# izhengfan/se2lam

Hardware: AMD Instinct MI355X
Metric: BA GN-iters/s (200 KF, 20k pts) (higher is better)
Workload: dtype f64; 1 GPU; globalBA-window 200 KF / 20000 landmarks / 119817 EdgeSE2XYZ + 199 PreEdgeSE2, LM optimize(10) (config 4 formulation, SURVEY D3); parallelism=single GPU

## Files before the change

### include/se2gpu.h

```cpp
#ifndef SE2GPU_H
#define SE2GPU_H

#include <stddef.h>
#include <stdint.h>

#ifdef __cplusplus
extern "C" {
#endif

#define SE2GPU_OK 0
#define SE2GPU_ERR_INVALID (-1)
#define SE2GPU_ERR_NO_DEVICE (-2)
#define SE2GPU_ERR_HIP (-3)
#define SE2GPU_ERR_CAPACITY (-4)
#define SE2GPU_ERR_STATE (-5)

const char* se2gpu_last_error(void);
int se2gpu_device_count(void);
const char* se2gpu_version(void);

typedef struct se2gpu_orb se2gpu_orb;

typedef struct se2gpu_orb_params {
    int32_t nfeatures;
// ... 247 lines not shown
                                  int* n_local, int32_t* ref_kfs, int* n_ref, int32_t* local_mps, int* n_mps);

int se2gpu_ba_initialize(se2gpu_ba* h);
int se2gpu_ba_set_edge_level(se2gpu_ba* h, int edge, int level);
int se2gpu_ba_reset_estimates(se2gpu_ba* h);
int se2gpu_ba_reset_estimates_batch(se2gpu_ba** handles, int count);

#define SE2GPU_BA_LM 0
#define SE2GPU_BA_GN 1
int se2gpu_ba_optimize(se2gpu_ba* h, int iters, int mode, const volatile uint8_t* stop_flag, int verbose,
                       se2gpu_ba_stats* stats);
int se2gpu_ba_optimize_batch(se2gpu_ba** handles, int count, int iters, int mode, const volatile uint8_t* stop_flag,
                             se2gpu_ba_stats* stats);
int se2gpu_ba_last_batch_path(void);
int se2gpu_ba_get_se2(se2gpu_ba* h, int id, double xyt[3]);
int se2gpu_ba_get_xyz(se2gpu_ba* h, int id, double xyz[3]);
int se2gpu_ba_get_all(se2gpu_ba* h, double* poses , double* lms );
double se2gpu_ba_chi2(se2gpu_ba* h);

int se2gpu_ba_debug_reduced_system(se2gpu_ba* h, double lambda, double* S, double* bs);
int se2gpu_ba_debug_solve(se2gpu_ba* h, double lambda, double* x, int* factor_ok);
int se2gpu_ba_debug_solver_path(const se2gpu_ba* h);
int se2gpu_ba_debug_linearize_counts(const se2gpu_ba* h, int* runs, int* skips, long long* twin_bytes);
int se2gpu_ba_debug_pool_sizes(int out2[2]);
int se2gpu_ba_debug_chol_verify(se2gpu_ba* h, unsigned long long* counts2, unsigned long long* records, int cap);
int se2gpu_ba_debug_solve_plan(int P, int D, const uint8_t* pattern, int allow_nd, int* nsys, int* nbc, int* depth, int* ntask,
                               int* ndep, int32_t* pose_off, int32_t* tasks4, int task_cap, int32_t* deps, int dep_cap);
int se2gpu_ba_debug_solve_plan_tile(int P, int D, const uint8_t* pattern, int allow_nd, int tile, int* nsys, int* nbc, int* depth, int* ntask,
                                    int* ndep, int32_t* pose_off, int32_t* tasks4, int task_cap, int32_t* deps, int dep_cap);
int se2gpu_ba_debug_solve_plan_neager(int P, int D, const uint8_t* pattern, int allow_nd, int tile, int32_t* neager, int cap);
int se2gpu_ba_debug_plan_neager(se2gpu_ba* h, int* nsys, int* permuted, int* ntask, int32_t* neager, int cap);

int se2gpu_triangulate(int n, const se2gpu_keypoint* kps_ref, const se2gpu_keypoint* kps_cur, int n_cur,
                       int32_t* match_idx, const uint8_t* has_observation, const float* P_ref, const float* P_cur,
                       const float* Ocam, float lower_depth, float upper_depth, int min_degree, float* pos_out,
                       uint8_t* good_parallax, int* n_good, int* n_tracked_old);

typedef struct se2gpu_track se2gpu_track;
int se2gpu_track_create(se2gpu_track** out);
void se2gpu_track_destroy(se2gpu_track* h);
int se2gpu_track_fundamental_mask(se2gpu_track* h, const float* pt1, const float* pt2, int n, uint8_t* mask,
                                  int* n_inliers);
int se2gpu_track_remove_outliers(se2gpu_track* h, const se2gpu_keypoint* kps1, int n1, const se2gpu_keypoint* kps2,
                                 int n2, int32_t* matches, int* n_inliers);
int se2gpu_track_last_ransac(const se2gpu_track* h, int info[4]);
int se2gpu_track_set_stream(se2gpu_track* h, void* hip_stream);
// ... 131 lines not shown
```

### se2lam_amd/capi.py

```python
from __future__ import annotations

import ctypes as C
import os

import numpy as np

HERE = os.path.dirname(os.path.abspath(__file__))
LIB_PATH = os.path.join(HERE, "lib", "libse2gpu.so")

OK = 0
ERR_INVALID, ERR_NO_DEVICE, ERR_HIP, ERR_CAPACITY, ERR_STATE = -1, -2, -3, -4, -5


class Se2GpuError(RuntimeError):
    def __init__(self, code, msg):
        super().__init__(f"se2gpu error {code}: {msg}")
        self.code = code


class Keypoint(C.Structure):
    _fields_ = [("x", C.c_float), ("y", C.c_float), ("size", C.c_float), ("angle", C.c_float),
                ("response", C.c_float), ("octave", C.c_int32), ("class_id", C.c_int32)]


# ... 145 lines not shown
    "se2gpu_ba_add_edge_se3": (_I, [_VP, _I, _I, _PD, _PD]),
    "se2gpu_ba_add_edge_xyz2uv": (_I, [_VP, _I, _I, _PD, _D, _D]),
    "se2gpu_ba_get_se3": (_I, [_VP, _I, _PD]),
    "se2gpu_ba_edge_chi2": (_I, [_VP, _PD, _I]),
    "se2gpu_map_update_local_graph": (_I, [C.POINTER(MapView), _I, _I, _VP, C.POINTER(_I), _VP, C.POINTER(_I), _VP, C.POINTER(_I)]),
    "se2gpu_sparsify_se3xyz": (_I, [_I, _VP, _VP, _VP, _VP, _VP, _VP, _VP, _VP, _VP]),
    "se2gpu_feat_edge_batch": (_I, [_I, _I, _I, _I, _VP, _VP, _D, _D, _D, _VP, _VP, _VP, _VP, _D, _D, _VP, _VP, _VP, _VP, _VP,
                                    _VP, _VP, _VP]),
    "se2gpu_ba_initialize": (_I, [_VP]),
    "se2gpu_ba_set_edge_level": (_I, [_VP, _I, _I]),
    "se2gpu_ba_reset_estimates": (_I, [_VP]),
    "se2gpu_ba_reset_estimates_batch": (_I, [_VP, _I]),
    "se2gpu_ba_optimize": (_I, [_VP, _I, _I, _PU8, _I, C.POINTER(BaStats)]),
    "se2gpu_ba_optimize_batch": (_I, [C.POINTER(_VP), _I, _I, _I, _PU8, C.POINTER(BaStats)]),
    "se2gpu_ba_last_batch_path": (_I, []),
    "se2gpu_ba_get_se2": (_I, [_VP, _I, _PD]),
    "se2gpu_ba_get_xyz": (_I, [_VP, _I, _PD]),
    "se2gpu_ba_get_all": (_I, [_VP, _PD, _PD]),
    "se2gpu_ba_chi2": (_D, [_VP]),
    "se2gpu_ba_debug_reduced_system": (_I, [_VP, _D, _PD, _PD]),
    "se2gpu_ba_debug_solve": (_I, [_VP, _D, _PD, C.POINTER(C.c_int)]),
    "se2gpu_ba_debug_solver_path": (_I, [_VP]),
    "se2gpu_ba_debug_linearize_counts": (_I, [_VP, C.POINTER(C.c_int), C.POINTER(C.c_int), C.POINTER(C.c_longlong)]),
    "se2gpu_ba_debug_chol_verify": (_I, [_VP, _VP, _VP, _I]),
    "se2gpu_ba_debug_pool_sizes": (_I, [_VP]),
    "se2gpu_ba_debug_solve_plan": (_I, [_I, _I, _VP, _I, _VP, _VP, _VP, _VP, _VP, _VP, _VP, _I, _VP, _I]),
    "se2gpu_ba_debug_solve_plan_tile": (_I, [_I, _I, _VP, _I, _I, _VP, _VP, _VP, _VP, _VP, _VP, _VP, _I, _VP, _I]),
    "se2gpu_ba_debug_solve_plan_neager": (_I, [_I, _I, _VP, _I, _I, _VP, _I]),
    "se2gpu_ba_debug_plan_neager": (_I, [_VP, C.POINTER(C.c_int), C.POINTER(C.c_int), C.POINTER(C.c_int), _VP, _I]),
    "se2gpu_triangulate": (_I, [_I, _VP, _VP, _I, _VP, _VP, _VP, _VP, _VP, C.c_float, C.c_float, _I, _VP, _VP,
                           C.POINTER(C.c_int), C.POINTER(C.c_int)]),
    "se2gpu_track_create": (_I, [C.POINTER(_VP)]),
    "se2gpu_track_destroy": (None, [_VP]),
    "se2gpu_track_fundamental_mask": (_I, [_VP, _VP, _VP, _I, _VP, C.POINTER(C.c_int)]),
    "se2gpu_track_remove_outliers": (_I, [_VP, _VP, _I, _VP, _I, _VP, C.POINTER(C.c_int)]),
    "se2gpu_track_last_ransac": (_I, [_VP, _VP]),
    "se2gpu_track_set_stream": (_I, [_VP, _VP]),
    "se2gpu_track_stream": (_VP, [_VP]),
    "se2gpu_track_sync": (_I, [_VP]),
    "se2gpu_track_loop_verify_batch_device": (_I, [_VP, _VP, _VP, _I, _I, _VP, _VP, _VP, _VP, _I, _VP, _VP, _VP, _VP]),
    "se2gpu_plane_motion_prior": (_I, [_VP, _VP, _D, _D, _D, _VP, _VP]),
    "se2gpu_track_pose_ba": (_I, [_VP, _VP, _VP, _VP, _I, _VP, _VP, _VP, _D, _D, _D, _D, _I, _VP, C.POINTER(BaStats)]),
    "se2gpu_track_triangulate": (_I, [_VP, _I, _VP, _VP, _I, _VP, _VP, _VP, _VP, _VP, C.c_float, C.c_float, _I, _VP, _VP,
                                 C.POINTER(C.c_int), C.POINTER(C.c_int)]),
    "se2gpu_ba_reduce_buffer_doubles": (_SZ, [_VP, _I]),
    "se2gpu_ba_exchange_doubles": (_SZ, [_I]),
# ... 214 lines not shown
```

### se2lam_amd/csrc/ba.hip

```cpp
#include <algorithm>
#include <atomic>
#include <chrono>
#include <cmath>
#include <cstdlib>
#include <functional>
#include <limits>
#include <mutex>
#include <thread>
#include <memory>
#include <unordered_map>

#include "common.h"
#include "se3_math.h"
#include "ba_device.h"
#include "ba3_device.h"
#include "ba_window.h"

using namespace se2gpu;
using namespace se2gpu::badev;

namespace {



// ... 1395 lines not shown
                                                     const int* __restrict__ col_src) {
    if (ctl && ctl->done) return;
    const int r = blockIdx.x * 4 + threadIdx.x / 64;
    const int lane = threadIdx.x & 63;
    if (r >= n) return;
    const double* y = A + (size_t)n * ld;
    double acc = 0.0;
    for (int c = r + lane; c < n; c += 64) acc += R[(size_t)r * ld + c] * y[c];
    acc = wave_sum(acc);
    const int dst = col_src ? col_src[r] : r;
    if (lane == 0 && dst >= 0) x[dst] = acc;
}

struct TrialEnd {
    double* out;
    volatile double* mail;
    double seq;
    BaCtl* ctl;
    const volatile int* stop;
    int step;
    int decide;
    int notify;
    int spec;
};

struct FinArgs {
    int enabled, nblk, P, O, root;
    const uint8_t* fixed;
    const double* xp;
    const double* bp;
    const double* poses;
    double* poses_trial;
    const int* o_i;
    const int* o_j;
    const double* o_meas;
    const double* o_info;
    unsigned* counter;
    TrialEnd te;
};
__device__ void finish_trial(const FinArgs& fin, const double* part, double lambda, double* fsp);

struct SpecArgs {
    RecSet set[2];
    double *Hpp_e, *bp_e;
};

// ... 169 lines not shown
        for (int i = 0; i < kBlock / 64; ++i) { c += sm[0][i]; s += sm[1][i]; }
        if (a.fin.enabled) {
            store_agent(a.part + 2 * bx, d2_t{c, s});
            asm volatile("s_waitcnt vmcnt(0)" ::: "memory");
            __hip_atomic_fetch_add(a.fin.counter, 1u, __ATOMIC_RELAXED, __HIP_MEMORY_SCOPE_AGENT);
        } else {
            a.part[2 * bx] = c;
            a.part[2 * bx + 1] = s;
        }
    }
    if (LIN && spec)
        lin_landmark<true>(l, sub, beg, end, a.L, hll, bsum, lambda_spec, keep, wr.W, a.sp.Hpp_e, a.sp.bp_e, wr.Hll, wr.bl, wr.Ainv,
                           wr.zeta, wr.Dg);
}
template <bool LIN>
__global__ __launch_bounds__(kBlock) void k_update(UpdArgs a) {
    d_update<LIN>(blockIdx.x, a);
}

__global__ void k_ctl_clear_error(BaCtl* __restrict__ ctl) {
    ctl->error = 0;
    ctl->done = 0;
}

__device__ inline void post_ctl(const BaCtl* c, volatile double* mail, double seq, int tid, int nthr) {
    constexpr int kWords = (int)(sizeof(BaCtl) / 8);
    const double* src = reinterpret_cast<const double*>(c);
    for (int i = tid; i < kWords; i += nthr) mail[8 + i] = src[i];
}

__device__ inline void end_slot(BaCtl* ctl, volatile double* mail, bool post, int tid, int nthr, bool step) {
    if (!step) return;
    if (tid == 0) ctl->seq += 1.0;
    __syncthreads();
    if (post && mail) {
        __threadfence();
        post_ctl(ctl, mail, 0.0, tid, nthr);
        __threadfence_system();
        __syncthreads();
        if (tid == 0) mail[kMailSeq] = ctl->seq;
    }
}


struct TrialState { bool live, est_b; double lambda; };
__device__ __forceinline__ TrialState trial_open(const TrialEnd& t, double lambda) {
// ... 24 lines not shown
    __syncthreads();
    if (threadIdx.x == 0)
        for (int w = 1; w < nw; ++w) {
            chi += sm[w];
            scale += sm[nw + w];
        }
}

__device__ __forceinline__ bool trial_decide(const TrialEnd& t, double chi, double scale, double fail, bool stopped, bool records) {
    BaCtl* ctl = t.ctl;
    volatile double* mail = t.mail;
    t.out[0] = chi; t.out[1] = scale; t.out[3] = 0;
    if (!t.step) t.out[2] = 0;
    if (ctl && t.decide) {
        if (!t.step) {
            lm_begin(ctl, chi, stopped);
        } else {
            const double sc[3] = {chi, scale, fail};
            const int sel0 = ctl->sel;
            const bool speculated = t.spec && ctl->it + 1 < ctl->iters;
            const double lambda_spec = lm_lambda_spec(ctl->lambda, ctl->mode);
            lm_advance(ctl, sc, stopped);
            if (records && !ctl->error) lm_records_advance(ctl, speculated, sel0, lambda_spec);
        }
        return (ctl->done || t.notify) && mail;
    }
    if (mail && !ctl) {
        mail[0] = chi;
        mail[1] = scale;
        mail[2] = fail;
        __threadfence_system();
        mail[3] = t.seq;
    }
    return false;
}

__device__ __forceinline__ void trial_close(const TrialEnd& t, const int* post) {
    if (!(t.ctl && t.decide)) return;
    __syncthreads();
    end_slot(t.ctl, t.mail, *post != 0, threadIdx.x, blockDim.x, t.step != 0);
}

__device__ __forceinline__ void se2_pose_stage(const FinArgs& fin, const double* poses, double* poses_trial, double lambda,
                                               bool step, double* sp, double& scale) {
    for (int p = threadIdx.x; p < fin.P; p += blockDim.x) {
        double x = poses[3 * p], y = poses[3 * p + 1], th = poses[3 * p + 2];
// ... 966 lines not shown
    hipEvent_t join_event = nullptr;
    hipStream_t join_stream = nullptr;
    bool own_pending = false;
    int P = 0, L = 0, E = 0, O = 0, nblk = 0, nparts = 0;
    int ld = 0;
    bool host_solve = false;
    DevBuf<double> poses0, lms0, poses_a, poses_b, lms_a, lms_b;
    double *poses = nullptr, *poses_t = nullptr, *lms = nullptr, *lms_t = nullptr;
    DevBuf<uint8_t> fixed;
    DevBuf<int> lm_ptr, e_kf, e_lm, pose_ptr, pose_edges, podo_ptr, podo_item, o_i, o_j;
    DevBuf<int> blk_a, blk_b, blk_ptr, pair_i, pair_j, blk_odo;
    DevBuf<int4> grp;
    int nwg_off = 0, grp_cap_wg = 0;
    DevBuf<uint8_t> garena;
    DevBuf<int> plan_np, plan_base, plan_key0, plan_key1, plan_idx, plan_hist, plan_offs, plan_out, plan_tsum, plan_toff;
    DevBuf<int2> plan_st0, plan_st1;
    bool odo_fallback = false;
    bool odo_self_loop = false;
    DevBuf<double> e_uv, e_info, o_meas, o_info;
    DevBuf<double> Hpl, Hpp_e, bp_e, Hll, bl, Dinv, z, Y, Dg, Hpp, bp, Oii, Ojj, Oij, obi, obj;
    DevBuf<double> red_own, xp, part, scal, diag3, Rinv;
    DevBuf<double> rec_twin;
    bool run_spec = false;
    DevBuf<double> red_packed;
    DevBuf<int4> chol_tasks;
    DevBuf<int> chol_deps;
    DevBuf<int> chol_neager;
    DevBuf<int> pose_off;
    DevBuf<int> col_src;
    std::vector<int> h_pose_off;
    DevBuf<uint8_t> plan_nz;
    DevBuf<double> plan_nzd;
    PinBuf<uint8_t> h_plan_nz;
    DevBuf<uint8_t> solver_arena;
    int nsys = 0;
    int solve_depth = 0;
    DevBuf<unsigned> chol_flags;
    DevBuf<unsigned long long> chol_head;
    DevBuf<unsigned long long> chol_vfy;
    DevBuf<int> plan_place;
    DevBuf<unsigned> fin_counter;
    DevBuf<unsigned long long> l0_acc;
    int chol_ntask = 0;
    struct GraphSlot { int iters = -1, mode = -1; hipGraphExec_t exec = nullptr; unsigned long stamp = 0; };
    static constexpr int kGraphSlots = 3;
    GraphSlot graphs[kGraphSlots];
    unsigned long graph_clock = 0;
    void drop_graphs() {
        for (auto& g : graphs) {
            if (g.exec) (void)hipGraphExecDestroy(g.exec);
            g = GraphSlot{};
        }
    }
    double dev_seq = 0;
    DevBuf<long long> chol_trace;
    bool chol_steps = false;
    bool chol_faulted = false;
    bool chol_fallback = false;
    double* red = nullptr;
    PinBuf<double> h_red, h_x, h_scal;
    double* h_mail = nullptr;
    double* d_mail = nullptr;
    volatile int* h_stop = nullptr;
    int* d_stop = nullptr;
    uint64_t mail_seq = 0;
    DevBuf<BaCtl> ctl;
    int run_mode = SE2GPU_BA_LM, run_iters = 0, run_enqueued = 0;
// ... 1132 lines not shown
            hipLaunchKernelGGL(k_plan_place, dim3(kPackRuns), dim3(128), 0, st, nblk, h->blk_a.p, h->blk_b.p, h->blk_ptr.p, start,
                               h->grp.p, cap_wg, gpw);
        } else {
            hipLaunchKernelGGL(k_plan_pack, dim3(1), dim3(256), 0, st, nblk, h->blk_a.p, h->blk_b.p, h->blk_ptr.p, h->grp.p,
                               cap_wg, h->plan_out.p, gpw);
        }
        SE2_HIP(hipGetLastError());
        SE2_CHECK(h->h_scal.reserve(8 + (size_t)h->world));
        SE2_HIP(hipMemcpyAsync(h->h_scal.p, h->plan_out.p, sizeof(int), hipMemcpyDeviceToHost, st));
        lap("plan kernels enqueued");
    }
    sent = big_off;
    SE2_CHECK(stage_range(big_off, big_end, copy_stream));
    SE2_HIP(hipEventRecord(h->ev_copy1, copy_stream));
    lap("measurements staged");
    SE2_HIP(hipStreamWaitEvent(st, h->ev_copy1, 0));
    SE2_CHECK(h->fin_counter.reserve(1));
    SE2_HIP(hipMemsetAsync(h->fin_counter.p, 0, sizeof(unsigned), st));
    SE2_CHECK(h->l0_acc.reserve(2));
    SE2_HIP(hipMemsetAsync(h->l0_acc.p, 0, 2 * sizeof(unsigned long long), st));
    SE2_HIP(hipMemsetAsync(h->ctl.p, 0, sizeof(BaCtl), st));
    h->dev_seq = 0;
    h->drop_graphs();
    SE2_CHECK(h->h_x.reserve(n));
    SE2_CHECK(h->h_scal.reserve(8 + (size_t)h->world));
    if (!h->h_mail) {
        SE2_HIP(hipHostMalloc((void**)&h->h_mail, kMailDoubles * sizeof(double), hipHostMallocMapped | hipHostMallocCoherent));
        std::memset(h->h_mail, 0, kMailDoubles * sizeof(double));
        SE2_HIP(hipHostGetDevicePointer((void**)&h->d_mail, h->h_mail, 0));
        h->h_stop = reinterpret_cast<volatile int*>(h->h_mail + kMailStop);
        h->d_stop = reinterpret_cast<int*>(h->d_mail + kMailStop);
    }
    ((volatile double*)h->h_mail)[kMailSeq] = 0.0;
    h->poses = h->poses_a.p; h->poses_t = h->poses_b.p;
    h->lms = h->lms_a.p; h->lms_t = h->lms_b.p;
    SE2_HIP(hipMemcpyAsync(h->poses, h->poses0.p, (size_t)ps * P * 8, hipMemcpyDeviceToDevice, st));
    if (L) SE2_HIP(hipMemcpyAsync(h->lms, h->lms0.p, 3 * (size_t)L * 8, hipMemcpyDeviceToDevice, st));
    if (pattern_early) SE2_HIP(hipEventSynchronize(h->ev_pat));
    else SE2_HIP(hipStreamSynchronize(st));
    lap(pattern_early ? "pattern" : "synchronise");
    {
        std::vector<uint8_t> pat;
        if (nd_possible) {
            const uint8_t* nz = device_plan ? h->h_plan_nz.p : pl.blk_nz.data();
            pat.assign((size_t)P * P, 0);
            for (int a = 0; a < P; ++a) {
// ... 112 lines not shown
    if (i < np) poses[i] = poses0[i];
    if (i < nl) lms[i] = lms0[i];
}
__global__ __launch_bounds__(256) void k_reset_batch(const ResetItem* __restrict__ items) {
    const ResetItem it = items[blockIdx.y];
    const unsigned stride = gridDim.x * 256, t0 = blockIdx.x * 256 + threadIdx.x;
    for (unsigned i = t0; i < it.np; i += stride) it.dst_p[i] = it.src_p[i];
    for (unsigned i = t0; i < it.nl; i += stride) it.dst_l[i] = it.src_l[i];
}

struct Bufs {
    const BaCtl* c;
    double *pa, *pb, *la, *lb;
};
inline Bufs bufs(se2gpu_ba* h, bool ctl) {
    if (ctl) return Bufs{h->ctl.p, h->poses_a.p, h->poses_b.p, h->lms_a.p, h->lms_b.p};
    return Bufs{nullptr, h->poses, h->poses_t, h->lms, h->lms_t};
}

bool ba_env_speculate() {
    static const bool on = env_flag("SE2GPU_BA_SPECULATE", true);
    return on;
}
bool ba_env_open() {
    static const bool on = env_flag("SE2GPU_BA_OPEN", true);
    return on;
}
bool ba_opens_fused(const se2gpu_ba* h) {
    return ba_env_open() && h->model == 0 && !h->allreduce && !h->comm && h->L > 0 && !h->odo_fallback;
}
RecSet rec_own(const se2gpu_ba* h) { return RecSet{h->Hpl.p, h->Dg.p, h->Hll.p, h->bl.p, h->Dinv.p, h->z.p}; }
RecSet rec_twin(const se2gpu_ba* h) {
    if (!h->rec_twin.p || h->model) return RecSet{};
    const size_t E = (size_t)h->E, L = (size_t)h->L;
    double* p = h->rec_twin.p;
    RecSet r;
    r.W = p; p += 9 * E + 1;
    r.Dg = p; p += 12 * E + 1;
    r.Hll = p; p += 6 * L + 1;
    r.bl = p; p += 3 * L + 1;
    r.Ainv = p; p += 6 * L + 1;
    r.zeta = p;
    return r;
}
int ba_reserve_twin(se2gpu_ba* h) { return h->rec_twin.reserve(21 * (size_t)h->E + 18 * (size_t)h->L + 6); }

// ... 13 lines not shown
    return PoseReduceArgs{h->P, h->pose_ptr.p, h->pose_edges.p, h->Hpp_e.p, h->bp_e.p, h->podo_ptr.p, h->podo_item.p, h->Oii.p,
                          h->Ojj.p, h->obi.p, h->obj.p, h->Hpp.p, h->bp.p};
}
MaxdiagArgs maxdiag_args(se2gpu_ba* h, int dpp, int stride9, BaCtl* ctl) {
    return MaxdiagArgs{h->L, h->Hll.p, h->P, stride9 ? h->Hpp.p : h->diag3.p, h->fixed.p, h->scal.p, dpp, stride9, ctl};
}
Reduce2Args reduce2_args(se2gpu_ba* h, const Bufs& B, double lambda, const RecSet& alt) {
    return Reduce2Args{h->P, h->ld, h->nwg_off, lambda, h->root, h->grp.p, h->blk_a.p, h->blk_b.p, h->pair_i.p, h->pair_j.p,
                       h->blk_odo.p, h->Hpl.p, h->Dg.p, h->fixed.p, h->pose_ptr.p, h->pose_edges.p, h->podo_ptr.p, h->podo_item.p,
                       h->o_i.p, h->o_j.p, h->o_meas.p, h->o_info.p, B.pa, h->red, h->bp.p, B.c, B.pb, &h->ctl.p->epoch,
                       h->pose_off.p, h->nsys, alt.W, alt.Dg};
}
CholArgs chol_args(se2gpu_ba* h, const BaCtl* ctl, int skip, unsigned long long* head, bool verify) {
    const int n = h->nsys, ld = h->ld;
    const int nt = ld / kNB, nbc = (n + kNB - 1) / kNB;
    double* YU = h->Rinv.p + 2 * (size_t)nt * nbc * kSlabs * kSlabDoubles;
    unsigned* flagA = h->chol_flags.p;
    return CholArgs{h->red, h->Rinv.p, YU, ld, n, nbc, h->chol_tasks.p + skip, h->chol_deps.p, h->chol_neager.p + skip, h->col_src.p,
                    flagA, flagA + kSlabs * (size_t)nt * nbc, &h->ctl.p->epoch, ba_scal(h) + 2, h->chol_trace.p, ctl, h->xp.p,
                    verify ? h->chol_vfy.p : nullptr, head, h->chol_ntask - skip};
}
TrialEnd trial_end(se2gpu_ba* h, const Bufs& B, int step, int decide, int notify, double seq, bool lin = false, bool post = true) {
    return TrialEnd{ba_scal(h), post ? h->d_mail : nullptr, seq, B.c ? h->ctl.p : nullptr,
                    B.c ? (const volatile int*)h->d_stop : nullptr, step, decide, notify, lin ? 1 : 0};
}
FinArgs fin_args(se2gpu_ba* h, const Bufs& B, const double* xp, const TrialEnd& te) {
    return FinArgs{1, (int)upd_grid(h).x, h->P, h->O, h->root, h->fixed.p, xp, h->bp.p, B.pa, B.pb,
                   h->o_i.p, h->o_j.p, h->o_meas.p, h->o_info.p, h->fin_counter.p, te};
}
UpdArgs upd_args(se2gpu_ba* h, const Bufs& B, double lambda, const double* xp, const FinArgs& fin, bool lin = false) {
    return UpdArgs{h->cam, h->L, lambda, h->lm_ptr.p, h->e_kf.p, h->e_uv.p, h->e_info.p, B.pa, h->fixed.p, B.la, xp, h->z.p, h->Hpl.p,
                   h->bl.p, B.lb, h->part.p, B.c, B.pb, fin, h->Dinv.p,
                   lin ? SpecArgs{{rec_own(h), rec_twin(h)}, h->Hpp_e.p, h->bp_e.p} : SpecArgs{}};
}

inline const double* prior_hess(const se2gpu_ba* h) { return h->model == 2 ? h->ph.p : h->prior_info.p; }
inline Edges6 edges6(const se2gpu_ba* h) {
    if (h->model == 2) return Edges6{h->pg_edges, h->pe_i.p, h->pe_j.p, h->pe_meas.p, h->pe_info.p};
    return Edges6{h->O, h->o_i.p, h->o_j.p, h->o_meas.p, h->o_info.p};
}
inline dim3 terms6_grid(const se2gpu_ba* h) { return grid1((size_t)h->P + h->O, 64); }
Lin3Args lin3_args(se2gpu_ba* h, const Bufs& B, double lambda) {
    return Lin3Args{h->cam3, h->L, h->lm_ptr.p, h->e_kf.p, h->e_uv.p, h->e_info.p, B.pa, h->fixed.p, B.la, h->Hpl.p, h->Hpp_e.p,
                    h->bp_e.p, h->Hll.p, h->bl.p, lambda, h->Dinv.p, h->z.p, h->Y.p, h->Dg.p, B.c, B.pb, B.lb};
}
Terms6Args terms6_args(se2gpu_ba* h, const Bufs& B) {
    return Terms6Args{h->P, h->O, B.pa, h->fixed.p, h->prior_has.p, h->prior_meas.p, h->prior_info.p, h->ph.p, h->pb.p, h->slot_a.p,
// ... 323 lines not shown
    };
    if (first && ba_opens_fused(h)) {
        const OpenArgs oa = open_args(h, B, lm, seq);
        if (lm) {
            SE2_LAUNCH(h->prof, st, "k_open", k_open<false>, open_grid(h, oa, true), dim3(kBlock), 0, oa);
            SE2_CHECK(ba_lambda_init(h, &oa.fin));
            SE2_CHECK(ba_reduce(h, 0.0, 3, true));
        } else {
            SE2_LAUNCH(h->prof, st, "k_open", k_open<true>, open_grid(h, oa, false), dim3(kBlock), 0, oa);
            SE2_CHECK(ba_reduce(h, 0.0, 0, true));
        }
        SE2_HIP(hipGetLastError());
    } else if (first) {
        SE2_CHECK(evaluate(false, false));
        if (lm) {
            SE2_CHECK(ba_linearize(h, -1.0, true));
            SE2_CHECK(ba_lambda_init(h));
            SE2_CHECK(ba_reduce(h, 0.0, 3, true));
        } else {
            SE2_CHECK(ba_linearize(h, 0.0, true));
            SE2_CHECK(ba_reduce(h, 0.0, 0, true));
        }
    } else {
        if (know_retry != 1) SE2_CHECK(ba_linearize(h, 0.0, true));
        SE2_CHECK(ba_reduce(h, 0.0, !lm ? 0 : know_retry == 0 ? 0 : know_retry == 1 ? 3 : (h->model ? 2 : 0), true));
    }
    SE2_CHECK(ba_allreduce_system(h));
    SE2_CHECK(ba_solve(h, true));
    SE2_CHECK(evaluate(true, notify));
    return SE2GPU_OK;
}


template <typename Args>
struct Packed {
    int nblk;
    Args args;
};
template <typename Args, void (*Body)(unsigned, const Args&), int BS>
__global__ __launch_bounds__(BS) void k_batched(const Packed<Args>* __restrict__ p) {
    if ((int)blockIdx.x >= p[blockIdx.y].nblk) return;
    const Args a = p[blockIdx.y].args;
    Body(blockIdx.x, a);
}
template <typename Args, void (*Body)(unsigned, const Args&), int BS>
__global__ __launch_bounds__(BS) void k_batched_xcd(const Packed<Args>* __restrict__ p) {
    const unsigned nb = gridDim.x, nw8 = gridDim.y & ~7u;
// ... 892 lines not shown
    return SE2GPU_OK;
}

int se2gpu_ba_debug_pool_sizes(int out2[2]) {
    SE2_REQUIRE(out2, SE2GPU_ERR_INVALID, "debug_pool_sizes: NULL argument");
    { LeasePool<PlanSet>& p = LeasePool<PlanSet>::get(); std::lock_guard<std::mutex> g(p.mu); out2[0] = (int)p.idle.size(); }
    { LeasePool<ResetScratch>& p = LeasePool<ResetScratch>::get(); std::lock_guard<std::mutex> g(p.mu); out2[1] = (int)p.idle.size(); }
    return SE2GPU_OK;
}

int se2gpu_ba_debug_solver_path(const se2gpu_ba* h) {
    if (!h || !h->initialized) return -1;
    return h->host_solve ? 3 : h->chol_fallback ? 2 : h->chol_steps ? 1 : 0;
}

int se2gpu_ba_debug_linearize_counts(const se2gpu_ba* h, int* runs, int* skips, long long* twin_bytes) {
    SE2_REQUIRE(h && h->initialized, SE2GPU_ERR_STATE, "debug_linearize_counts before initialize");
    BaCtl c;
    std::memset(&c, 0, sizeof(c));
    if (h->h_mail && !h->run_active) std::memcpy(&c, (const void*)(h->h_mail + 8), sizeof(BaCtl));
    if (runs) *runs = c.lin_runs;
    if (skips) *skips = c.lin_skips;
    if (twin_bytes) *twin_bytes = (long long)(h->rec_twin.cap * sizeof(double));
    return SE2GPU_OK;
}

int se2gpu_ba_debug_solve(se2gpu_ba* h, double lambda, double* x, int* factor_ok) {
    SE2_REQUIRE(h && h->initialized && x, SE2GPU_ERR_STATE, "debug_solve before initialize");
    SE2_CHECK(ba_join(h));
    const int n = h->D * h->P;
    SE2_CHECK(ba_linearize(h, lambda));
    SE2_CHECK(ba_reduce(h, lambda, false));
    SE2_CHECK(ba_allreduce(h, h->red, (size_t)(h->nsys + 1) * h->ld));
    SE2_CHECK(ba_solve(h));
    SE2_HIP(hipStreamSynchronize(h->stream));
    SE2_HIP(hipMemcpy(x, h->xp.p, (size_t)n * 8, hipMemcpyDeviceToHost));
    double f = 0;
    SE2_HIP(hipMemcpy(&f, h->red + (size_t)h->ld * h->ld + 2, 8, hipMemcpyDeviceToHost));
    SE2_REQUIRE(f < 1e5, SE2GPU_ERR_HIP, "k_chol_tiles: a dependency spin timed out (2 s)");
    if (factor_ok) *factor_ok = !(f > 0.0);
    if (h->chol_trace.p && !h->chol_steps) {
        std::vector<long long> tr(16 * (size_t)h->chol_ntask);
        std::vector<int4> tk(h->chol_ntask);
        SE2_HIP(hipMemcpy(tr.data(), h->chol_trace.p, tr.size() * sizeof(long long), hipMemcpyDeviceToHost));
        SE2_HIP(hipMemcpy(tk.data(), h->chol_tasks.p, tk.size() * sizeof(int4), hipMemcpyDeviceToHost));
        int ndep = 0;
// ... 16 lines not shown
            if ((tk[t].x >> 16) == 2 || ne[t] < 2) continue;
            std::fprintf(stderr, "choleager %d", t);
            for (int q = tk[t].w - ne[t]; q < tk[t].w; ++q) std::fprintf(stderr, " %d", dp[q]);
            std::fprintf(stderr, "\n");
        }
    }
    return SE2GPU_OK;
}

namespace {

bool ba_env_sync() {
    static const bool on = env_flag("SE2GPU_BA_SYNC", false);
    return on;
}

int ba_run_prologue(se2gpu_ba* h, hipStream_t st, hipEvent_t* ev, int iters, int mode, bool sync, const volatile uint8_t* stop_flag) {
    SE2_CHECK(ba_join(h, st, ev));
    h->est_valid = false;
    h->run_mode = mode;
    h->run_iters = iters;
    h->run_enqueued = 0;
    h->run_sync = sync;
    h->run_spec = false;
    h->run_active = true;
    *h->h_stop = (stop_flag && *stop_flag) ? 1 : 0;
    return SE2GPU_OK;
}

int ba_run_begin(se2gpu_ba* h, int iters, int mode, const volatile uint8_t* stop_flag, int verbose) {
    SE2_REQUIRE(h && h->initialized, SE2GPU_ERR_STATE, "optimize before initialize");
    SE2_REQUIRE(mode == SE2GPU_BA_LM || mode == SE2GPU_BA_GN, SE2GPU_ERR_INVALID, "unknown mode %d", mode);
    SE2_REQUIRE(h->d_mail, SE2GPU_ERR_STATE, "SE2GPU_BA_MAILBOX=0 is no longer supported: the LM controller posts its state "
                                              "through the mapped mailbox");
    const bool sync = ba_env_sync() || h->prof.enabled || verbose || h->odo_fallback || h->host_solve;
    SE2_CHECK(ba_run_prologue(h, h->stream, nullptr, iters, mode, sync, stop_flag));
    h->run_spec = ba_env_speculate() && h->model == 0 && !h->allreduce && !h->comm && h->L > 0 && iters > 1;
    if (h->run_spec) SE2_CHECK(ba_reserve_twin(h));
    const int n0 = h->run_sync ? 1 : std::max(iters, 1);
    auto enqueue_all = [&]() -> int {
        hipLaunchKernelGGL(k_ctl_init, dim3(1), dim3(64), 0, h->stream, CtlInitArgs{h->ctl.p, iters, mode});
        SE2_HIP(hipGetLastError());
        for (int k = 0; k < n0; ++k) SE2_CHECK(ba_enqueue_trial(h, k == 0, h->run_sync ? 0 : -1, k == n0 - 1, 0.0));
        return SE2GPU_OK;
    };
    static const bool graphs_on = env_flag("SE2GPU_BA_GRAPH", true);
    const bool graphable = graphs_on && !h->run_sync && !h->allreduce && !h->comm && iters > 0;
    se2gpu_ba::GraphSlot* slot = nullptr;
    if (graphable) {
        for (auto& g : h->graphs)
            if (g.iters == iters && g.mode == mode) slot = &g;
        if (!slot) {
            slot = &h->graphs[0];
            for (auto& g : h->graphs)
                if (g.stamp < slot->stamp) slot = &g;
            if (slot->exec) (void)hipGraphExecDestroy(slot->exec);
            *slot = se2gpu_ba::GraphSlot{};
            slot->iters = iters;
            slot->mode = mode;
            slot->stamp = ++h->graph_clock;
            SE2_CHECK(enqueue_all());
        } else if (slot->exec) {
            slot->stamp = ++h->graph_clock;
            SE2_HIP(hipGraphLaunch(slot->exec, h->stream));
        } else {
            slot->stamp = ++h->graph_clock;
            hipGraph_t g = nullptr;
            SE2_HIP(hipStreamBeginCapture(h->stream, hipStreamCaptureModeThreadLocal));
            const int rc = enqueue_all();
            const hipError_t ce = hipStreamEndCapture(h->stream, &g);
            SE2_CHECK(rc);
            SE2_HIP(ce);
            const hipError_t ie = hipGraphInstantiate(&slot->exec, g, nullptr, nullptr, 0);
            (void)hipGraphDestroy(g);
            SE2_HIP(ie);
            SE2_HIP(hipGraphLaunch(slot->exec, h->stream));
        }
    } else {
        SE2_CHECK(enqueue_all());
    }
    h->dev_seq += n0;
    h->run_seq = h->dev_seq;
    h->run_enqueued = n0;
    return SE2GPU_OK;
}

int ba_run_step(se2gpu_ba* h, bool wait, const volatile uint8_t* stop_flag, int verbose, int* finished) {
    *finished = 0;
    if (stop_flag && *stop_flag) *h->h_stop = 1;
    const double first = h->run_seq - h->run_enqueued;
    if (wait) SE2_CHECK(ba_wait_seq(h, kMailSeq, h->run_seq, first, &h, 1, stop_flag, 30, "the LM controller never reported back"));
    else if (!ba_mail_at(h, kMailSeq, h->run_seq, first)) return SE2GPU_OK;
    std::atomic_thread_fence(std::memory_order_acquire);
    BaCtl c;
    std::memcpy(&c, (const void*)(h->h_mail + 8), sizeof(BaCtl));
    if (c.error && !h->chol_steps) {
        std::fprintf(stderr, "se2gpu_ba: k_chol_tiles timed out; continuing with k_chol_step\n");
        h->chol_steps = h->chol_fallback = true;
        h->drop_graphs();
        SE2_HIP(hipStreamSynchronize(h->stream));
        hipLaunchKernelGGL(k_ctl_clear_error, dim3(1), dim3(1), 0, h->stream, h->ctl.p);
        c.error = 0;
        c.done = 0;
        h->run_enqueued = 0;
        ((volatile double*)h->h_mail)[kMailSeq] = 0.0;
    }
    SE2_REQUIRE(!c.error, SE2GPU_ERR_HIP, "k_chol_step: the factorisation reported a time-out");
    if (verbose)
        fprintf(stderr, "se2gpu_ba: it %d trial %d chi2 %.9g rho %.3g lambda %.6g%s\n", c.it, c.qmax, c.current_chi, c.rho,
                c.lambda, c.retry ? " (rejected)" : "");
    if (h->run_sync)
        if ((h->poses == h->poses_b.p) != (c.sel != 0)) { std::swap(h->poses, h->poses_t); std::swap(h->lms, h->lms_t); }
    if (c.done) {
        *finished = 1;
        return SE2GPU_OK;
    }
    const int more = h->run_sync ? 1 : std::max(1, c.iters - c.it);
    for (int k = 0; k < more; ++k) {
        SE2_CHECK(ba_enqueue_trial(h, false, h->run_sync ? (c.retry ? 1 : 0) : -1, k == more - 1, 0.0));
        h->dev_seq += 1;
        h->run_seq = h->dev_seq;
        ++h->run_enqueued;
    }
    return SE2GPU_OK;
}

int ba_run_finish(se2gpu_ba* h, se2gpu_ba_stats* stats) {
    h->own_pending = false;
// ... 274 lines not shown
            for (int k = 0; k < more; ++k) SE2_CHECK(ba_batch_slot(*g.bp, false, k == more - 1));
            for (int i = 0; i < g.count; ++i) {
                g.hs[i]->dev_seq += more;
                g.hs[i]->run_seq = g.hs[i]->dev_seq;
                g.hs[i]->run_enqueued += more;
            }
        }
    }
    for (int i = 0; i < count; ++i) SE2_CHECK(ba_run_finish(hs[i], stats ? stats + i : nullptr));
    return SE2GPU_OK;
}

}

int se2gpu_ba_optimize(se2gpu_ba* h, int iters, int mode, const volatile uint8_t* stop_flag, int verbose,
                       se2gpu_ba_stats* stats) {
    SE2_CHECK(ba_run_begin(h, iters, mode, stop_flag, verbose));
    for (int fin = 0; !fin;) SE2_CHECK(ba_run_step(h, true, stop_flag, verbose, &fin));
    return ba_run_finish(h, stats);
}

static int ba_optimize_group(se2gpu_ba** hs, int count, int iters, int mode, const volatile uint8_t* stop_flag,
                             se2gpu_ba_stats* stats) {
    for (int i = 0; i < count; ++i) SE2_CHECK(ba_run_begin(hs[i], iters, mode, stop_flag, 0));
    std::vector<char> fin(count, 0);
    int left = count;
    const auto t0 = std::chrono::steady_clock::now();
    long spins = 0;
    while (left) {
        for (int i = 0; i < count; ++i) {
            if (fin[i]) continue;
            int f = 0;
            SE2_CHECK(ba_run_step(hs[i], hs[i]->run_sync, stop_flag, 0, &f));
            if (f) { fin[i] = 1; --left; }
        }
        __builtin_ia32_pause();
        if ((++spins & 0xfffff) == 0 && std::chrono::steady_clock::now() - t0 > std::chrono::seconds(60))
            for (int i = 0; i < count; ++i)
                if (!fin[i]) { int f = 0; SE2_CHECK(ba_run_step(hs[i], true, stop_flag, 0, &f)); if (f) { fin[i] = 1; --left; } }
    }
    for (int i = 0; i < count; ++i) SE2_CHECK(ba_run_finish(hs[i], stats ? stats + i : nullptr));
    return SE2GPU_OK;
}

static thread_local int t_last_batch_path = -1;
int se2gpu_ba_last_batch_path(void) { return t_last_batch_path; }

// ... 161 lines not shown
```

### se2lam_amd/csrc/ba_device.h

```cpp
#pragma once
#include <hip/hip_runtime.h>

#include <cmath>

#include "../../include/se2gpu.h"

namespace se2gpu {
namespace badev {

constexpr int kGroup = 8;
constexpr int kBlock = 256;
constexpr double kPi = 3.14159265358979323846;

struct CamDev {
    double fx, cx, cy;
    double Rcb[9];
    double tcb[3];
    double huber;
};

constexpr int kMailSeq = 4;
struct BaCtl {
    double lambda, ni, current_chi, rho;
    double chi2_init, chi2_final;
    int it, qmax, trials, iters;
    int done, terminated, stopped, retry;
    int sel;
    int mode, error, pad;
    double chi2_hist[64], lambda_hist[64];
    int trials_hist[64];
    int rec_sel, rec_valid, lin_runs, lin_skips;
    double seq;
    unsigned epoch;
    unsigned pad2;
};

__host__ __device__ inline double normalize_theta(double theta) {
    if (theta >= -kPi && theta < kPi) return theta;
    double multiplier = floor(theta / (2 * kPi));
    theta = theta - multiplier * 2 * kPi;
    if (theta >= kPi) theta -= 2 * kPi;
    if (theta < -kPi) theta += 2 * kPi;
    return theta;
}

template <bool JAC>
__device__ inline void se2xyz(const CamDev& cam, double px, double py, double pth, double lx, double ly, double lz,
                              double u, double v, double& e0, double& e1, double* Jp, double* Jl) {
    double s, c;
    sincos(pth, &s, &c);
    const double dx = lx - px, dy = ly - py;
// ... 163 lines not shown
```

### se2lam_amd/optimizer.py

```python
from __future__ import annotations

import ctypes as C
import os

import numpy as np

from . import capi

LM, GN = 0, 1


def _stats_dict(st):
    n = min(st.iterations, 64)
    return dict(iterations=st.iterations, trials=st.trials, terminated=bool(st.terminated),
                stopped=bool(st.stopped), chi2_init=st.chi2_init, chi2_final=st.chi2_final,
                lambda_final=st.lambda_final, chi2_hist=list(st.chi2_hist[:n]),
                lambda_hist=list(st.lambda_hist[:n]), trials_hist=list(st.trials_hist[:n]))


def _no_fallback(h):
    if capi.lib().se2gpu_ba_debug_solver_path(h) == 2 and os.environ.get("SE2GPU_BA_CHOL_FAULT") != "1":
        raise RuntimeError("se2gpu_ba: k_chol_tiles timed out and the handle fell back to k_chol_step")


# ... 70 lines not shown
    def exchange_doubles(self) -> int:
        return int(capi.lib().se2gpu_ba_exchange_doubles_h(self._h))

    def chol_verify(self):
        counts = np.zeros(2, np.uint64)
        rec = np.zeros((64, 8), np.uint64)
        capi.check(capi.lib().se2gpu_ba_debug_chol_verify(self._h, counts.ctypes.data, rec.ctypes.data, 64))
        return int(counts[0]), int(counts[1]), rec[:min(int(counts[0]), 64)]

    def plan_neager(self):
        nsys, perm, ntask = C.c_int(0), C.c_int(0), C.c_int(0)
        capi.check(capi.lib().se2gpu_ba_debug_plan_neager(self._h, C.byref(nsys), C.byref(perm), C.byref(ntask), None, 0))
        ne = np.zeros(max(ntask.value, 1), np.int32)
        capi.check(capi.lib().se2gpu_ba_debug_plan_neager(self._h, C.byref(nsys), C.byref(perm), C.byref(ntask), ne.ctypes.data, len(ne)))
        return int(nsys.value), bool(perm.value), ne[:ntask.value]

    def solver_path(self) -> int:
        return int(capi.lib().se2gpu_ba_debug_solver_path(self._h))

    def linearize_counts(self):
        runs, skips, twin = C.c_int(0), C.c_int(0), C.c_longlong(0)
        capi.check(capi.lib().se2gpu_ba_debug_linearize_counts(self._h, C.byref(runs), C.byref(skips), C.byref(twin)))
        return int(runs.value), int(skips.value), int(twin.value)

    def activeRobustChi2(self) -> float:
        v = capi.lib().se2gpu_ba_chi2(self._h)
        if v < 0:
            capi.check(capi.ERR_STATE)
        return float(v)

    def load(self, g):
        l = capi.lib()
        capi.check(l.se2gpu_ba_add_cam(self._h, g.fx, g.cx, g.cy))
        R = np.ascontiguousarray(g.Rbc, np.float64).reshape(-1)
        t = np.ascontiguousarray(g.tbc, np.float64).reshape(-1)
        capi.check(l.se2gpu_ba_set_Tbc(self._h, capi.pd(R), capi.pd(t)))
        a = [np.ascontiguousarray(g.poses, np.float64), np.ascontiguousarray(g.fixed, np.uint8),
             np.ascontiguousarray(g.lms, np.float64), np.ascontiguousarray(g.e_kf, np.int32),
             np.ascontiguousarray(g.e_lm, np.int32), np.ascontiguousarray(g.e_uv, np.float64),
             np.ascontiguousarray(g.e_info, np.float64), np.ascontiguousarray(g.o_i, np.int32),
             np.ascontiguousarray(g.o_j, np.int32), np.ascontiguousarray(g.o_meas, np.float64),
             np.ascontiguousarray(g.o_info, np.float64)]
        P32, PU8 = C.POINTER(C.c_int32), C.POINTER(C.c_uint8)
        capi.check(l.se2gpu_ba_load(self._h, g.P, g.L, g.E, g.O, capi.pd(a[0]), a[1].ctypes.data_as(PU8),
                                    capi.pd(a[2]), a[3].ctypes.data_as(P32), a[4].ctypes.data_as(P32),
                                    capi.pd(a[5]), capi.pd(a[6]), a[7].ctypes.data_as(P32),
# ... 289 lines not shown
```

Before: 7378 iters/s.

## Drop host-side linearization gate on speculative runs with halt-and-resume fallback

On non-batch, async speculative runs, the host no longer enqueues a mandatory linearize pass before each trial. Instead the device controller halts the run whenever the speculative record turns out invalid, and the host then resumes it with a fresh linearize path. A cooldown counter disables the ungated mode for several runs after a halt, and cached graphs are keyed by the ungated flag. The aim is to save the linearize work and the extra host round trip when speculation hits, at the cost of an extra resume launch and graph variant when it misses.

```diff
diff --git a/include/se2gpu.h b/include/se2gpu.h
--- a/include/se2gpu.h
+++ b/include/se2gpu.h
@@ -293,6 +293,8 @@
 int se2gpu_ba_debug_solve(se2gpu_ba* h, double lambda, double* x, int* factor_ok);
 int se2gpu_ba_debug_solver_path(const se2gpu_ba* h);
 int se2gpu_ba_debug_linearize_counts(const se2gpu_ba* h, int* runs, int* skips, long long* twin_bytes);
+int se2gpu_ba_debug_gate_counts(const se2gpu_ba* h, int out3[3]);
+int se2gpu_ba_debug_set_gate_cooldown(se2gpu_ba* h, int runs);
 int se2gpu_ba_debug_pool_sizes(int out2[2]);
 int se2gpu_ba_debug_chol_verify(se2gpu_ba* h, unsigned long long* counts2, unsigned long long* records, int cap);
 int se2gpu_ba_debug_solve_plan(int P, int D, const uint8_t* pattern, int allow_nd, int* nsys, int* nbc, int* depth, int* ntask,
diff --git a/se2lam_amd/capi.py b/se2lam_amd/capi.py
--- a/se2lam_amd/capi.py
+++ b/se2lam_amd/capi.py
@@ -191,6 +191,8 @@
     "se2gpu_ba_debug_solve": (_I, [_VP, _D, _PD, C.POINTER(C.c_int)]),
     "se2gpu_ba_debug_solver_path": (_I, [_VP]),
     "se2gpu_ba_debug_linearize_counts": (_I, [_VP, C.POINTER(C.c_int), C.POINTER(C.c_int), C.POINTER(C.c_longlong)]),
+    "se2gpu_ba_debug_gate_counts": (_I, [_VP, C.POINTER(C.c_int)]),
+    "se2gpu_ba_debug_set_gate_cooldown": (_I, [_VP, _I]),
     "se2gpu_ba_debug_chol_verify": (_I, [_VP, _VP, _VP, _I]),
     "se2gpu_ba_debug_pool_sizes": (_I, [_VP]),
     "se2gpu_ba_debug_solve_plan": (_I, [_I, _I, _VP, _I, _VP, _VP, _VP, _VP, _VP, _VP, _VP, _I, _VP, _I]),
diff --git a/se2lam_amd/csrc/ba.hip b/se2lam_amd/csrc/ba.hip
--- a/se2lam_amd/csrc/ba.hip
+++ b/se2lam_amd/csrc/ba.hip
@@ -1441,6 +1441,7 @@
     int decide;
     int notify;
     int spec;
+    int ungated;
 };
 
 struct FinArgs {
@@ -1656,6 +1657,10 @@
     ctl->error = 0;
     ctl->done = 0;
 }
+__global__ void k_ctl_resume(BaCtl* __restrict__ ctl) {
+    ctl->halted = 0;
+    ctl->done = 0;
+}
 
 __device__ inline void post_ctl(const BaCtl* c, volatile double* mail, double seq, int tid, int nthr) {
     constexpr int kWords = (int)(sizeof(BaCtl) / 8);
@@ -1726,6 +1731,7 @@
             const double lambda_spec = lm_lambda_spec(ctl->lambda, ctl->mode);
             lm_advance(ctl, sc, stopped);
             if (records && !ctl->error) lm_records_advance(ctl, speculated, sel0, lambda_spec);
+            if (t.ungated && !ctl->done && !ctl->error && !ctl->rec_valid) { ctl->halted = 1; ctl->done = 1; }
         }
         return (ctl->done || t.notify) && mail;
     }
@@ -2738,6 +2744,10 @@
     DevBuf<double> red_own, xp, part, scal, diag3, Rinv;
     DevBuf<double> rec_twin;
     bool run_spec = false;
+    bool run_ungated = false;
+    static constexpr int kGateCooldown = 8;
+    int gate_cooldown = 0, gate_cooldown_runs = kGateCooldown;
+    int gate_ungated_runs = 0, gate_halts = 0;
     DevBuf<double> red_packed;
     DevBuf<int4> chol_tasks;
     DevBuf<int> chol_deps;
@@ -2758,7 +2768,7 @@
     DevBuf<unsigned> fin_counter;
     DevBuf<unsigned long long> l0_acc;
     int chol_ntask = 0;
-    struct GraphSlot { int iters = -1, mode = -1; hipGraphExec_t exec = nullptr; unsigned long stamp = 0; };
+    struct GraphSlot { int iters = -1, mode = -1; bool ungated = false; hipGraphExec_t exec = nullptr; unsigned long stamp = 0; };
     static constexpr int kGraphSlots = 3;
     GraphSlot graphs[kGraphSlots];
     unsigned long graph_clock = 0;
@@ -3937,6 +3947,8 @@
     SE2_HIP(hipMemsetAsync(h->ctl.p, 0, sizeof(BaCtl), st));
     h->dev_seq = 0;
     h->drop_graphs();
+    h->gate_cooldown = h->gate_ungated_runs = h->gate_halts = 0;
+    h->gate_cooldown_runs = se2gpu_ba::kGateCooldown;
     SE2_CHECK(h->h_x.reserve(n));
     SE2_CHECK(h->h_scal.reserve(8 + (size_t)h->world));
     if (!h->h_mail) {
@@ -4095,6 +4107,10 @@
     static const bool on = env_flag("SE2GPU_BA_SPECULATE", true);
     return on;
 }
+bool ba_env_gate() {
+    static const bool on = env_flag("SE2GPU_BA_GATE", false);
+    return on;
+}
 bool ba_env_open() {
     static const bool on = env_flag("SE2GPU_BA_OPEN", true);
     return on;
@@ -4154,7 +4170,8 @@
 }
 TrialEnd trial_end(se2gpu_ba* h, const Bufs& B, int step, int decide, int notify, double seq, bool lin = false, bool post = true) {
     return TrialEnd{ba_scal(h), post ? h->d_mail : nullptr, seq, B.c ? h->ctl.p : nullptr,
-                    B.c ? (const volatile int*)h->d_stop : nullptr, step, decide, notify, lin ? 1 : 0};
+                    B.c ? (const volatile int*)h->d_stop : nullptr, step, decide, notify, lin ? 1 : 0,
+                    lin && h->run_ungated ? 1 : 0};
 }
 FinArgs fin_args(se2gpu_ba* h, const Bufs& B, const double* xp, const TrialEnd& te) {
     return FinArgs{1, (int)upd_grid(h).x, h->P, h->O, h->root, h->fixed.p, xp, h->bp.p, B.pa, B.pb,
@@ -4524,7 +4541,7 @@
             SE2_CHECK(ba_reduce(h, 0.0, 0, true));
         }
     } else {
-        if (know_retry != 1) SE2_CHECK(ba_linearize(h, 0.0, true));
+        if (know_retry != 1 && !h->run_ungated) SE2_CHECK(ba_linearize(h, 0.0, true));
         SE2_CHECK(ba_reduce(h, 0.0, !lm ? 0 : know_retry == 0 ? 0 : know_retry == 1 ? 3 : (h->model ? 2 : 0), true));
     }
     SE2_CHECK(ba_allreduce_system(h));
@@ -5463,6 +5480,20 @@
     if (runs) *runs = c.lin_runs;
     if (skips) *skips = c.lin_skips;
     if (twin_bytes) *twin_bytes = (long long)(h->rec_twin.cap * sizeof(double));
+    return SE2GPU_OK;
+}
+
+int se2gpu_ba_debug_gate_counts(const se2gpu_ba* h, int out3[3]) {
+    SE2_REQUIRE(h && h->initialized && out3, SE2GPU_ERR_STATE, "debug_gate_counts before initialize");
+    out3[0] = h->gate_ungated_runs;
+    out3[1] = h->gate_halts;
+    out3[2] = h->gate_cooldown;
+    return SE2GPU_OK;
+}
+int se2gpu_ba_debug_set_gate_cooldown(se2gpu_ba* h, int runs) {
+    SE2_REQUIRE(h && h->initialized && runs >= 0, SE2GPU_ERR_STATE, "debug_set_gate_cooldown: before initialize, or a negative count");
+    h->gate_cooldown_runs = runs;
+    h->gate_cooldown = std::min(h->gate_cooldown, runs);
     return SE2GPU_OK;
 }
 
@@ -5525,13 +5556,13 @@
     h->run_iters = iters;
     h->run_enqueued = 0;
     h->run_sync = sync;
-    h->run_spec = false;
+    h->run_spec = h->run_ungated = false;
     h->run_active = true;
     *h->h_stop = (stop_flag && *stop_flag) ? 1 : 0;
     return SE2GPU_OK;
 }
 
-int ba_run_begin(se2gpu_ba* h, int iters, int mode, const volatile uint8_t* stop_flag, int verbose) {
+int ba_run_begin(se2gpu_ba* h, int iters, int mode, const volatile uint8_t* stop_flag, int verbose, bool batch = false) {
     SE2_REQUIRE(h && h->initialized, SE2GPU_ERR_STATE, "optimize before initialize");
     SE2_REQUIRE(mode == SE2GPU_BA_LM || mode == SE2GPU_BA_GN, SE2GPU_ERR_INVALID, "unknown mode %d", mode);
     SE2_REQUIRE(h->d_mail, SE2GPU_ERR_STATE, "SE2GPU_BA_MAILBOX=0 is no longer supported: the LM controller posts its state "
@@ -5540,6 +5571,10 @@
     SE2_CHECK(ba_run_prologue(h, h->stream, nullptr, iters, mode, sync, stop_flag));
     h->run_spec = ba_env_speculate() && h->model == 0 && !h->allreduce && !h->comm && h->L > 0 && iters > 1;
     if (h->run_spec) SE2_CHECK(ba_reserve_twin(h));
+    h->run_ungated = h->run_spec && !h->run_sync && !batch && !ba_env_gate() && h->gate_cooldown == 0;
+    if (h->run_ungated) ++h->gate_ungated_runs;
+    else if (h->gate_cooldown > 0) --h->gate_cooldown;
+    const bool ungated = h->run_ungated;
     const int n0 = h->run_sync ? 1 : std::max(iters, 1);
     auto enqueue_all = [&]() -> int {
         hipLaunchKernelGGL(k_ctl_init, dim3(1), dim3(64), 0, h->stream, CtlInitArgs{h->ctl.p, iters, mode});
@@ -5552,7 +5587,7 @@
     se2gpu_ba::GraphSlot* slot = nullptr;
     if (graphable) {
         for (auto& g : h->graphs)
-            if (g.iters == iters && g.mode == mode) slot = &g;
+            if (g.iters == iters && g.mode == mode && g.ungated == ungated) slot = &g;
         if (!slot) {
             slot = &h->graphs[0];
             for (auto& g : h->graphs)
@@ -5561,6 +5596,7 @@
             *slot = se2gpu_ba::GraphSlot{};
             slot->iters = iters;
             slot->mode = mode;
+            slot->ungated = ungated;
             slot->stamp = ++h->graph_clock;
             SE2_CHECK(enqueue_all());
         } else if (slot->exec) {
@@ -5607,6 +5643,16 @@
         c.done = 0;
         h->run_enqueued = 0;
         ((volatile double*)h->h_mail)[kMailSeq] = 0.0;
+        h->run_ungated = false;
+    }
+    if (c.done && c.halted) {
+        hipLaunchKernelGGL(k_ctl_resume, dim3(1), dim3(1), 0, h->stream, h->ctl.p);
+        SE2_HIP(hipGetLastError());
+        c.done = c.halted = 0;
+        h->run_enqueued = 0;
+        h->run_ungated = false;
+        h->gate_cooldown = h->gate_cooldown_runs;
+        ++h->gate_halts;
     }
     SE2_REQUIRE(!c.error, SE2GPU_ERR_HIP, "k_chol_step: the factorisation reported a time-out");
     if (verbose)
@@ -5927,7 +5973,7 @@
 
 static int ba_optimize_group(se2gpu_ba** hs, int count, int iters, int mode, const volatile uint8_t* stop_flag,
                              se2gpu_ba_stats* stats) {
-    for (int i = 0; i < count; ++i) SE2_CHECK(ba_run_begin(hs[i], iters, mode, stop_flag, 0));
+    for (int i = 0; i < count; ++i) SE2_CHECK(ba_run_begin(hs[i], iters, mode, stop_flag, 0, true));
     std::vector<char> fin(count, 0);
     int left = count;
     const auto t0 = std::chrono::steady_clock::now();
diff --git a/se2lam_amd/csrc/ba_device.h b/se2lam_amd/csrc/ba_device.h
--- a/se2lam_amd/csrc/ba_device.h
+++ b/se2lam_amd/csrc/ba_device.h
@@ -26,7 +26,8 @@
     int it, qmax, trials, iters;
     int done, terminated, stopped, retry;
     int sel;
-    int mode, error, pad;
+    int mode, error;
+    int halted;
     double chi2_hist[64], lambda_hist[64];
     int trials_hist[64];
     int rec_sel, rec_valid, lin_runs, lin_skips;
diff --git a/se2lam_amd/optimizer.py b/se2lam_amd/optimizer.py
--- a/se2lam_amd/optimizer.py
+++ b/se2lam_amd/optimizer.py
@@ -116,6 +116,14 @@
         runs, skips, twin = C.c_int(0), C.c_int(0), C.c_longlong(0)
         capi.check(capi.lib().se2gpu_ba_debug_linearize_counts(self._h, C.byref(runs), C.byref(skips), C.byref(twin)))
         return int(runs.value), int(skips.value), int(twin.value)
+
+    def gate_counts(self):
+        out = (C.c_int * 3)()
+        capi.check(capi.lib().se2gpu_ba_debug_gate_counts(self._h, out))
+        return int(out[0]), int(out[1]), int(out[2])
+
+    def set_gate_cooldown(self, runs: int):
+        capi.check(capi.lib().se2gpu_ba_debug_set_gate_cooldown(self._h, int(runs)))
 
     def activeRobustChi2(self) -> float:
         v = capi.lib().se2gpu_ba_chi2(self._h)
```

Result: no change. 7445 iters/s, median of 6 (+0.9%).
